# Ighina/MultimodalTopicSegmentation

Measured on AMD Instinct MI355X. Metric: sentences/sec (fwd+bwd), higher is better.
Workload: dtype bf16; 1 GPU; BASELINE configs[1]: restricted-window transformer tagger d=1792 heads=8 ff=256 radius=15 layers=1 focal loss, 64 docs x 256 sentences per GPU, fwd+bwd+Adam(eps 1e-7), inputs resident in HBM; global_batch_docs=64, sentences_per_doc=256, parallelism=dp1 (document-sharded, RCCL all-reduce)

## Files before the change

multimodaltopicsegmentation_amd/csrc/ffn_fused.hip:

```cpp
#include <algorithm>
#include "gemm_common.h"

#define FF_BM 64
#define FF_F 256
#define FF_IMG 32768
#define FF_RING (FF_IMG)
#define FF_A_STAGE (8192 + 32768)
#define FF_B_STAGE 32768
#define FF_LDS (FF_IMG + 4 * FF_B_STAGE)
#ifdef FFN_STAMPS
#define FSTAMP(i) do { const unsigned long long t_ = __builtin_amdgcn_s_memtime(); tacc[i] += t_ - tprev; tprev = t_; } while (0)
#else
#define FSTAMP(i) do { } while (0)
#endif

struct FfnArgs {
  const bf16_t* X;
  const bf16_t* Wa;
  const bf16_t* Wb;
  const float* ba;
  const float* bb;
  const bf16_t* U;
  bf16_t* Uout;
  bf16_t* T;
  bf16_t* Y;
  int M, D, relu;
#ifdef FFN_STAMPS
  unsigned long long* stamps;
#endif
};

__device__ __forceinline__ int ff_col(int j, int n) { return (j >> 1) * 32 + (n >> 2) * 8 + (j & 1) * 4 + (n & 3); }

template <bool PERM>
__device__ __forceinline__ void ff_piece_kmajor(const bf16_t* __restrict__ G, int ld, int row0, int dim, int k0, char* img, int piece, int lane) {
  const int row = piece * 8 + (lane >> 3), pos = lane & 7;
  const int ch = pos ^ ((row >> 1) & 7);
  const int srow = PERM ? (row & ~63) + ff_col((row >> 4) & 3, row & 15) : row;
  const bf16_t* src = G + (size_t)min(row0 + srow, dim - 1) * ld + k0 + ch * 8;
  __builtin_amdgcn_global_load_lds((gptr_t*)src, (lptr_t*)(img + piece * 1024), 16, 0, 0);
}
__device__ __forceinline__ void ff_piece_strided(const bf16_t* __restrict__ G, int ld, int k0, int col0, char* img, int piece, int lane) {
  const int kr = piece * 4 + (lane >> 4), c16 = lane & 15;
  const int ch = ((((c16 >> 1) ^ strided_key(kr))) << 1) | (c16 & 1);
  const bf16_t* src = G + (size_t)(k0 + kr) * ld + col0 + ch * 8;
  __builtin_amdgcn_global_load_lds((gptr_t*)src, (lptr_t*)(img + piece * 1024), 16, 0, 0);
}

__device__ __forceinline__ frag_raw ff_frag_strided(const char* tile, int kbase, int wcol0, int j, int lane) {
  const int r = lane & 15, q = r >> 2, p = r & 3;
  const int col = wcol0 + (j >> 1) * 32 + (j & 1) * 4 + 8 * p;
  const unsigned addr = (unsigned)(uintptr_t)(__attribute__((address_space(3))) const char*)(tile + strided_off(kbase + q, col));
  frag_raw f;
  asm volatile("ds_read_b64_tr_b16 %0, %1" : "=v"(f.lo) : "v"(addr));
  asm volatile("ds_read_b64_tr_b16 %0, %1 offset:1024" : "=v"(f.hi) : "v"(addr));
  return f;
}

#define FF_CWAVES 8
#define FF_LWAVES 4
#define FF_THREADS ((FF_CWAVES + FF_LWAVES) * 64)

template <bool BWD>
__global__ __launch_bounds__(FF_THREADS) void ffn_fused_kernel(const FfnArgs a) {
  constexpr bool WKM = !BWD;
  extern __shared__ __attribute__((aligned(16))) char smem[];
  char* fimg = smem;
  char* ring = smem + FF_RING;
  const int tid = threadIdx.x, lane = tid & 63;
  const int wave = __builtin_amdgcn_readfirstlane(tid >> 6);
  const int bm0 = blockIdx.x * FF_BM;
  const int D = a.D, M = a.M;
  const int nkA = D / 64, nch = D / 256, nB = nch * 4;
#ifdef FFN_STAMPS
  unsigned long long tacc[16] = {0, 0, 0, 0, 0, 0, 0, 0, 0, 0, 0, 0, 0, 0, 0, 0};
  unsigned long long tprev = __builtin_amdgcn_s_memtime();
#define FF_STAMPS_OUT() do { if (a.stamps && lane == 0) for (int i_ = 0; i_ < 16; ++i_) a.stamps[((size_t)blockIdx.x * 12 + wave) * 16 + i_] = tacc[i_]; } while (0)
#else
#define FF_STAMPS_OUT() do { } while (0)
#endif

  if (wave >= FF_CWAVES) {
    const int lw = wave - FF_CWAVES;
    auto dmaA = [&](int kt) {
      char* st = ring + (kt % 3) * FF_A_STAGE;
#pragma unroll
      for (int i = 0; i < 10; ++i) {
        const int q = lw * 10 + i;
        if (q < 8) ff_piece_kmajor<false>(a.X, D, bm0, M, kt * 64, st, q, lane);
        else if constexpr (WKM) ff_piece_kmajor<true>(a.Wa, D, 0, FF_F, kt * 64, st + 8192, q - 8, lane);
        else ff_piece_strided(a.Wa, FF_F, kt * 64, ((q - 8) >> 4) * 128, st + 8192 + ((q - 8) >> 4) * 16384, (q - 8) & 15, lane);
      }
    };
    auto dmaB = [&](int gi) {
      char* st = ring + (gi & 3) * FF_B_STAGE;
      const int c = gi >> 2, kk = gi & 3;
#pragma unroll
      for (int i = 0; i < 8; ++i) {
        const int q = lw * 8 + i;
        if constexpr (WKM) ff_piece_kmajor<true>(a.Wb, FF_F, c * 256, D, kk * 64, st, q, lane);
        else ff_piece_strided(a.Wb, D, kk * 64, c * 256 + (q >> 4) * 128, st + (q >> 4) * 16384, q & 15, lane);
      }
    };
    dmaA(0);
    if (nkA > 1) { dmaA(1); asm volatile("s_waitcnt vmcnt(10)" ::: "memory"); }
    else asm volatile("s_waitcnt vmcnt(0)" ::: "memory");
    __builtin_amdgcn_s_barrier();
#pragma clang loop unroll(disable)
    for (int kt = 0; kt < nkA; ++kt) {
      if (kt + 2 < nkA) { dmaA(kt + 2); FSTAMP(0); asm volatile("s_waitcnt vmcnt(10)" ::: "memory"); }
      else asm volatile("s_waitcnt vmcnt(0)" ::: "memory");
      FSTAMP(3);
      __builtin_amdgcn_s_barrier();
      FSTAMP(4);
    }
    dmaB(0);
    dmaB(1);
    dmaB(2);
    dmaB(3);
    FSTAMP(5);
    asm volatile("s_waitcnt vmcnt(0)" ::: "memory");
    __builtin_amdgcn_s_barrier();
    FSTAMP(6);
#pragma clang loop unroll(disable)
    for (int gi = 0; gi < nB; ++gi) {
      if (gi >= 1 && gi + 3 < nB) { dmaB(gi + 3); FSTAMP(8); asm volatile("s_waitcnt vmcnt(16)" ::: "memory"); }
      else asm volatile("s_waitcnt vmcnt(0)" ::: "memory");
      FSTAMP(11);
      __builtin_amdgcn_s_barrier();
      FSTAMP(12);
    }
    FF_STAMPS_OUT();
    return;
  }

  const int wm = wave >> 2, wn = wave & 3;
  const int r16 = lane & 15, g = lane >> 4;
#ifdef FFN_STAMPS
  int tb = 0;
#endif
  f32x4 acc[2][4];
#pragma unroll
  for (int i = 0; i < 2; ++i)
#pragma unroll
    for (int j = 0; j < 4; ++j) acc[i][j] = (f32x4){0.f, 0.f, 0.f, 0.f};

  const unsigned lds0 = (unsigned)(uintptr_t)(__attribute__((address_space(3))) char*)smem;
  unsigned lk[2];
#pragma unroll
  for (int ks = 0; ks < 2; ++ks) lk[ks] = lds0 + r16 * 128 + (((ks * 4 + g) ^ ((r16 >> 1) & 7)) << 4);
  auto mma_tile = [&](int Aoff, int Boff) {
    LFrag<true> fa[2][2];
    LFrag<WKM> fb[4][2];
#pragma unroll
    for (int ks = 0; ks < 2; ++ks) {
      const unsigned ab = lk[ks] + Aoff + wm * 4096, bb = lk[ks] + Boff + wn * 8192;
#pragma unroll
      for (int j = 0; j < 4; ++j) {
        if constexpr (WKM) asm volatile("ds_read_b128 %0, %1 offset:%2" : "=v"(fb[j][ks].k) : "v"(bb), "n"(j * 2048));
        else fb[j][ks].s = ff_frag_strided(smem + Boff + (wn >> 1) * 16384, ks * 32 + 8 * g, (wn & 1) * 64, j, lane);
      }
#pragma unroll
      for (int i = 0; i < 2; ++i) asm volatile("ds_read_b128 %0, %1 offset:%2" : "=v"(fa[i][ks].k) : "v"(ab), "n"(i * 2048));
    }
    lgkm_wait<0>();
    FSTAMP(tb + 1);
    __builtin_amdgcn_s_setprio(1);
#pragma unroll
    for (int ks = 0; ks < 2; ++ks) {
      bf16x8 vb[4];
#pragma unroll
      for (int j = 0; j < 4; ++j) vb[j] = lfrag_get<WKM>(fb[j][ks]);
#pragma unroll
      for (int i = 0; i < 2; ++i) {
        const bf16x8 va = lfrag_get<true>(fa[i][ks]);
#pragma unroll
        for (int j = 0; j < 4; ++j) acc[i][j] = __builtin_amdgcn_mfma_f32_16x16x32_bf16(vb[j], va, acc[i][j], 0, 0, 0);
      }
    }
    __builtin_amdgcn_s_setprio(0);
    FSTAMP(tb + 2);
  };

  typedef __attribute__((ext_vector_type(4))) unsigned u32x4;
  uint4 upre[2][2];
  float4 b1[2][2];
  if constexpr (BWD) {
#pragma unroll
    for (int i = 0; i < 2; ++i)
#pragma unroll
      for (int h = 0; h < 2; ++h)
        upre[i][h] = *reinterpret_cast<const uint4*>(a.U + (size_t)min(bm0 + wm * 32 + i * 16 + r16, M - 1) * FF_F + wn * 64 + h * 32 + g * 8);
  } else {
#pragma unroll
    for (int h = 0; h < 2; ++h)
#pragma unroll
      for (int e = 0; e < 2; ++e) b1[h][e] = *reinterpret_cast<const float4*>(a.ba + wn * 64 + h * 32 + g * 8 + e * 4);
  }
  __builtin_amdgcn_s_barrier();
#pragma clang loop unroll(disable)
  for (int kt = 0; kt < nkA; ++kt) {
    FSTAMP(0);
    const int st = FF_RING + (kt % 3) * FF_A_STAGE;
    mma_tile(st, st + 8192);
    FSTAMP(3);
    __builtin_amdgcn_s_barrier();
    FSTAMP(4);
  }
#pragma unroll
  for (int i = 0; i < 2; ++i) {
    const int row = wm * 32 + i * 16 + r16;
#pragma unroll
    for (int h = 0; h < 2; ++h) {
      float v[8];
#pragma unroll
      for (int e = 0; e < 4; ++e) { v[e] = acc[i][2 * h][e]; v[4 + e] = acc[i][2 * h + 1][e]; }
      const size_t go = (size_t)(bm0 + row) * FF_F + wn * 64 + h * 32 + g * 8;
      if constexpr (!BWD) {
        v[0] += b1[h][0].x; v[1] += b1[h][0].y; v[2] += b1[h][0].z; v[3] += b1[h][0].w;
        v[4] += b1[h][1].x; v[5] += b1[h][1].y; v[6] += b1[h][1].z; v[7] += b1[h][1].w;
        uint4 pre;
        pre.x = pack_bf16x2(v[0], v[1]); pre.y = pack_bf16x2(v[2], v[3]); pre.z = pack_bf16x2(v[4], v[5]); pre.w = pack_bf16x2(v[6], v[7]);
        *reinterpret_cast<uint4*>(a.Uout + go) = pre;
#pragma unroll
        for (int r = 0; r < 8; ++r) v[r] = a.relu ? fmaxf(v[r], 0.0f) : gelu_erf_f(v[r]);
      } else {
        const unsigned uw[4] = {upre[i][h].x, upre[i][h].y, upre[i][h].z, upre[i][h].w};
#pragma unroll
        for (int r = 0; r < 8; ++r) {
          const float uu = (r & 1) ? bf16_hi(uw[r >> 1]) : bf16_lo(uw[r >> 1]);
          const float dr = to_f32(from_f32<bf16_t>(v[r]));
          v[r] = a.relu ? (uu > 0.0f ? dr : 0.0f) : dr * gelu_erf_grad_f(uu);
        }
      }
      uint4 t;
      t.x = pack_bf16x2(v[0], v[1]); t.y = pack_bf16x2(v[2], v[3]); t.z = pack_bf16x2(v[4], v[5]); t.w = pack_bf16x2(v[6], v[7]);
      *reinterpret_cast<uint4*>(a.T + go) = t;
      *reinterpret_cast<uint4*>(fimg + wn * 8192 + kmajor_off(row, h * 4 + g)) = t;
    }
#pragma unroll
    for (int j = 0; j < 4; ++j) acc[i][j] = (f32x4){0.f, 0.f, 0.f, 0.f};
  }
  FSTAMP(5);
  asm volatile("s_waitcnt lgkmcnt(0)" ::: "memory");
  __builtin_amdgcn_s_barrier();
  FSTAMP(6);
#ifdef FFN_STAMPS
  tb = 8;
#endif

  float4 b2[2][2];
  uint4 res[2][2];
#pragma clang loop unroll(disable)
  for (int c = 0; c < nch; ++c) {
    const int colw = c * 256 + wn * 64 + g * 8;
#pragma unroll
    for (int kk = 0; kk < 4; ++kk) {
      const int gi = c * 4 + kk;
      if (kk == 3) {
        if constexpr (!BWD) {
#pragma unroll
          for (int h = 0; h < 2; ++h)
#pragma unroll
            for (int e = 0; e < 2; ++e) b2[h][e] = *reinterpret_cast<const float4*>(a.bb + colw + h * 32 + e * 4);
        }
      }
      if (kk == 1) {
#pragma unroll
        for (int i = 0; i < 2; ++i)
#pragma unroll
          for (int h = 0; h < 2; ++h)
            res[i][h] = *reinterpret_cast<const uint4*>(a.X + (size_t)min(bm0 + wm * 32 + i * 16 + r16, M - 1) * D + colw + h * 32);
      }
      FSTAMP(8);
      mma_tile(kk * 8192, FF_RING + kk * FF_B_STAGE);
      if (kk == 3) {
#pragma unroll
        for (int i = 0; i < 2; ++i) {
          const int row = bm0 + wm * 32 + i * 16 + r16;
#pragma unroll
          for (int h = 0; h < 2; ++h) {
            float v[8];
#pragma unroll
            for (int e = 0; e < 4; ++e) { v[e] = acc[i][2 * h][e]; v[4 + e] = acc[i][2 * h + 1][e]; }
            if constexpr (!BWD) {
              v[0] += b2[h][0].x; v[1] += b2[h][0].y; v[2] += b2[h][0].z; v[3] += b2[h][0].w;
              v[4] += b2[h][1].x; v[5] += b2[h][1].y; v[6] += b2[h][1].z; v[7] += b2[h][1].w;
            }
            const unsigned rw[4] = {res[i][h].x, res[i][h].y, res[i][h].z, res[i][h].w};
#pragma unroll
            for (int e = 0; e < 4; ++e) { v[2 * e] += bf16_lo(rw[e]); v[2 * e + 1] += bf16_hi(rw[e]); }
            uint4 o;
            o.x = pack_bf16x2(v[0], v[1]); o.y = pack_bf16x2(v[2], v[3]); o.z = pack_bf16x2(v[4], v[5]); o.w = pack_bf16x2(v[6], v[7]);
            *reinterpret_cast<uint4*>(a.Y + (size_t)row * D + colw + h * 32) = o;
          }
#pragma unroll
          for (int j = 0; j < 4; ++j) acc[i][j] = (f32x4){0.f, 0.f, 0.f, 0.f};
        }
      }
      FSTAMP(11);
      __builtin_amdgcn_s_barrier();
      FSTAMP(12);
    }
  }
  FF_STAMPS_OUT();
}

#ifdef FFN_STAMPS
static unsigned long long* g_ffn_stamps = nullptr;
extern "C" void mts_ffn_set_stamps(void* p) { g_ffn_stamps = (unsigned long long*)p; }
#endif
static int ffn_launch(bool bwd, hipStream_t st, const FfnArgs& a0) {
  FfnArgs a = a0;
#ifdef FFN_STAMPS
  a.stamps = g_ffn_stamps;
#endif
  const int grid = ceil_div(a.M, FF_BM);
  if (bwd) {
    auto k = ffn_fused_kernel<true>;
    if (int rc = mts_dyn_lds(k, FF_LDS, "ffn_fused")) return rc;
    hipLaunchKernelGGL(k, dim3(grid), dim3(FF_THREADS), FF_LDS, st, a);
  } else {
    auto k = ffn_fused_kernel<false>;
    if (int rc = mts_dyn_lds(k, FF_LDS, "ffn_fused")) return rc;
    hipLaunchKernelGGL(k, dim3(grid), dim3(FF_THREADS), FF_LDS, st, a);
  }
  MTS_LAUNCH_CHECK("mts_ffn_fused");
  return MTS_OK;
}

static int ffn_check(const char* who, int M, int D, int F, const void* p0, const void* p1, const void* p2, const void* p3, const void* p4) {
  MTS_CHECK_ARG(M > 0 && p0 && p1 && p2 && p3 && p4, "%s: bad arguments", who);
  MTS_UNSUPPORTED(F == FF_F && D >= 256 && D % 256 == 0, "%s: the fused block covers F = 256 and D a multiple of 256 (F=%d, D=%d)", who, F, D);
  return MTS_OK;
}

extern "C" int mts_ffn_supported(int dtype, int M, int D, int F) { return dtype == MTS_BF16 && M > 0 && F == FF_F && D >= 256 && D % 256 == 0; }

extern "C" int mts_ffn_fwd(void* stream, int M, int D, int F, const void* a1, const void* w1, const float* b1, const void* w2, const float* b2,
                           int relu, void* u, void* f, void* s2) {
  if (int rc = ffn_check("mts_ffn_fwd", M, D, F, a1, w1, w2, s2, f)) return rc;
  MTS_CHECK_ARG(b1 && b2 && u, "mts_ffn_fwd: null bias / u");
  FfnArgs a{(const bf16_t*)a1, (const bf16_t*)w1, (const bf16_t*)w2, b1, b2, nullptr, (bf16_t*)u, (bf16_t*)f, (bf16_t*)s2, M, D, relu};
  return ffn_launch(false, (hipStream_t)stream, a);
}

extern "C" int mts_ffn_bwd_data(void* stream, int M, int D, int F, const void* ds2, const void* w1, const void* w2, const void* u, int relu,
                                void* du, void* da1) {
  if (int rc = ffn_check("mts_ffn_bwd_data", M, D, F, ds2, w1, w2, du, da1)) return rc;
  MTS_CHECK_ARG(u, "mts_ffn_bwd_data: null u");
  FfnArgs a{(const bf16_t*)ds2, (const bf16_t*)w2, (const bf16_t*)w1, nullptr, nullptr, (const bf16_t*)u, nullptr, (bf16_t*)du, (bf16_t*)da1, M, D, relu};
  return ffn_launch(true, (hipStream_t)stream, a);
}
```

multimodaltopicsegmentation_amd/csrc/gemm.hip:

```cpp
#include <algorithm>
#include <math.h>
#include <stdlib.h>
#include "common.h"

#include "gemm_common.h"


template <int LAYOUT, typename TC, bool GLDS>
__global__ __launch_bounds__(256, 2) void gemm_bf16_kernel(const GemmArgs a) {
  constexpr bool A_KMAJOR = (LAYOUT == MTS_NT || LAYOUT == MTS_NN);
  constexpr bool B_KMAJOR = (LAYOUT == MTS_NT || LAYOUT == MTS_TT);
  extern __shared__ __attribute__((aligned(16))) char smem[];

  const int tid = threadIdx.x;
  const int lane = tid & 63;
  const int wave = tid >> 6;
  const int wm = wave >> 1, wn = wave & 1;
  const int r16 = lane & 15, g = lane >> 4;

  const int ntn = (a.N + BN - 1) / BN;
  const int ntm = (a.M + BM - 1) / BM;
  const int nt = ntn * ntm;
  int bid = xcd_remap(blockIdx.x, nt);
  const int bm0 = (ntm < ntn ? bid % ntm : bid / ntn) * BM;
// ... 329 lines not shown
      float v[4] = {0.f, 0.f, 0.f, 0.f};
      if (kc) {
        const int row = r0 + (f >> 2), k = k0 + (f & 3) * 4;
        if (row < rdim) {
          const float* p = X + (long)row * sr + k;
          if (vec && k + 3 < kend) { const float4 t = *reinterpret_cast<const float4*>(p); v[0] = t.x; v[1] = t.y; v[2] = t.z; v[3] = t.w; }
          else for (int j = 0; j < 4; ++j) if (k + j < kend) v[j] = p[j];
        }
      } else {
        const int k = k0 + (f >> 5), row = r0 + (f & 31) * 4;
        if (k < kend) {
          const float* p = X + (long)k * sk + row;
          if (vec && row + 3 < rdim) { const float4 t = *reinterpret_cast<const float4*>(p); v[0] = t.x; v[1] = t.y; v[2] = t.z; v[3] = t.w; }
          else for (int j = 0; j < 4; ++j) if (row + j < rdim) v[j] = p[j];
        }
      }
      r[i] = make_float4(v[0], v[1], v[2], v[3]);
    }
  };
  auto store_op = [&](float (&S)[F32_BK][F32_PITCH], bool kc, const float4 (&r)[2]) {
#pragma unroll
    for (int i = 0; i < 2; ++i) {
      const int f = tid + 256 * i;
      if (kc) {
        const int row = f >> 2, k = (f & 3) * 4;
        S[k][row] = r[i].x; S[k + 1][row] = r[i].y; S[k + 2][row] = r[i].z; S[k + 3][row] = r[i].w;
      } else {
        *reinterpret_cast<float4*>(&S[f >> 5][(f & 31) * 4]) = r[i];
      }
    }
  };

  f32x4 acc[4][4];
#pragma unroll
  for (int i = 0; i < 4; ++i)
#pragma unroll
    for (int j = 0; j < 4; ++j) acc[i][j] = (f32x4){0.f, 0.f, 0.f, 0.f};

  const int nk = (kend - kbeg + F32_BK - 1) / F32_BK;
  load_op(A, s.sam, s.sak, a_kc, a_vec, bm0, a.M, kbeg, ra);
  load_op(B, s.sbn, s.sbk, b_kc, b_vec, bn0, a.N, kbeg, rb);
  store_op(As[0], a_kc, ra);
  store_op(Bs[0], b_kc, rb);
  __syncthreads();
  for (int kt = 0; kt < nk; ++kt) {
    const int buf = kt & 1;
    if (kt + 1 < nk) {
      load_op(A, s.sam, s.sak, a_kc, a_vec, bm0, a.M, kbeg + (kt + 1) * F32_BK, ra);
      load_op(B, s.sbn, s.sbk, b_kc, b_vec, bn0, a.N, kbeg + (kt + 1) * F32_BK, rb);
    }
#pragma unroll
    for (int ks = 0; ks < F32_BK / 4; ++ks) {
      float av[4], bv[4];
#pragma unroll
      for (int i = 0; i < 4; ++i) {
        av[i] = As[buf][ks * 4 + g][wm * 64 + i * 16 + r16];
        bv[i] = Bs[buf][ks * 4 + g][wn * 64 + i * 16 + r16];
      }
#pragma unroll
      for (int i = 0; i < 4; ++i)
#pragma unroll
        for (int j = 0; j < 4; ++j) acc[i][j] = __builtin_amdgcn_mfma_f32_16x16x4f32(bv[j], av[i], acc[i][j], 0, 0, 0);
    }
    if (kt + 1 < nk) {
      store_op(As[buf ^ 1], a_kc, ra);
      store_op(Bs[buf ^ 1], b_kc, rb);
    }
    __syncthreads();
  }
#pragma unroll
  for (int i = 0; i < 4; ++i) {
    const int m = bm0 + wm * 64 + i * 16 + r16;
#pragma unroll
    for (int j = 0; j < 4; ++j) {
      const int n = bn0 + wn * 64 + j * 16 + 4 * g;
      float v[4] = {acc[i][j][0], acc[i][j][1], acc[i][j][2], acc[i][j][3]};
      epilogue4<float, float>(a, m, n, v, true);
    }
  }
}

#define COLSUM_RS 128
template <typename T>
__global__ __launch_bounds__(256) void colsum_partial_kernel(const T* __restrict__ X, int M, int N, int ldx,
                                                             float* __restrict__ partial) {
  __shared__ float red[16][64];
  const int cx = threadIdx.x & 15, ry = threadIdx.x >> 4;
  const int n = blockIdx.x * 64 + cx * 4;
  const int rs = blockIdx.y;
  const int rows_per = (M + COLSUM_RS - 1) / COLSUM_RS;
  const int m0 = rs * rows_per, m1 = min(M, m0 + rows_per);
  float s[4] = {0.f, 0.f, 0.f, 0.f};
  if (n + 3 < N) {
    int m = m0 + ry;
    for (; m + 48 < m1; m += 64) {
      float v[4][4];
#pragma unroll
      for (int u = 0; u < 4; ++u) load4<T>(X + (size_t)(m + 16 * u) * ldx + n, v[u]);
#pragma unroll
      for (int u = 0; u < 4; ++u)
#pragma unroll
        for (int i = 0; i < 4; ++i) s[i] += v[u][i];
    }
    for (; m < m1; m += 16) {
      float v[4];
      load4<T>(X + (size_t)m * ldx + n, v);
#pragma unroll
      for (int i = 0; i < 4; ++i) s[i] += v[i];
    }
  } else if (n < N) {
    for (int m = m0 + ry; m < m1; m += 16)
      for (int i = 0; i < 4 && n + i < N; ++i) s[i] += to_f32(X[(size_t)m * ldx + n + i]);
  }
#pragma unroll
  for (int i = 0; i < 4; ++i) red[ry][cx * 4 + i] = s[i];
  __syncthreads();
  if (threadIdx.x < 64) {
    const int c = threadIdx.x, nn = blockIdx.x * 64 + c;
    float t = 0.f;
#pragma unroll
    for (int r = 0; r < 16; ++r) t += red[r][c];
    if (nn < N) partial[(size_t)rs * N + nn] = t;
  }
}
__global__ __launch_bounds__(256) void colsum_final_kernel(const float* __restrict__ partial, int N, int nparts,
                                                           float* __restrict__ out, int accumulate) {
  __shared__ float red[4][64];
  const int col = threadIdx.x & 63, grp = threadIdx.x >> 6;
  const int n = blockIdx.x * 64 + col;
  float s = 0.f;
  if (n < N) {
    int r = grp;
    for (; r + 4 * 7 < nparts; r += 4 * 8) {
      float v[8];
#pragma unroll
      for (int u = 0; u < 8; ++u) v[u] = partial[(size_t)(r + 4 * u) * N + n];
#pragma unroll
      for (int u = 0; u < 8; ++u) s += v[u];
    }
    for (; r < nparts; r += 4) s += partial[(size_t)r * N + n];
  }
  red[grp][col] = s;
  __syncthreads();
  if (grp == 0 && n < N) {
    const float t = (red[0][col] + red[1][col]) + (red[2][col] + red[3][col]);
    out[n] = accumulate ? out[n] + t : t;
  }
}

__global__ __launch_bounds__(256) void splitk_reduce_kernel(const float* __restrict__ slab, int splits, int M, int N, float* __restrict__ C,
                                                            int ldc, int accumulate) {
  const size_t idx = (size_t)blockIdx.x * 256 + threadIdx.x;
  const int n4 = N / 4;
  if (idx >= (size_t)M * n4) return;
  const int m = (int)(idx / n4), n = 4 * (int)(idx % n4);
  float s[4] = {0.f, 0.f, 0.f, 0.f};
  if (accumulate) load4<float>(C + (size_t)m * ldc + n, s);
  const size_t plane = (size_t)M * N;
  for (int z = 0; z < splits; ++z) {
    float v[4];
    load4<float>(slab + z * plane + (size_t)m * N + n, v);
#pragma unroll
    for (int i = 0; i < 4; ++i) s[i] += v[i];
  }
  store4<float>(C + (size_t)m * ldc + n, s);
}

__global__ __launch_bounds__(256) void splitk_reduce_t_kernel(const float* __restrict__ slab, int splits, int M, int N, float* __restrict__ Ct,
                                                              int ldc, int accumulate) {
  __shared__ float tile[32][33];
  const int n0 = blockIdx.x * 32, m0 = blockIdx.y * 32;
  const int tx = threadIdx.x & 31, ty = threadIdx.x >> 5;
  const size_t plane = (size_t)M * N;
#pragma unroll
  for (int r = ty; r < 32; r += 8) {
    const int m = m0 + r, n = n0 + tx;
    float s = 0.f;
    if (m < M && n < N) {
      const float* p = slab + (size_t)m * N + n;
      int z = 0;
      for (; z + 7 < splits; z += 8) {
        float v[8];
#pragma unroll
        for (int u = 0; u < 8; ++u) v[u] = p[(size_t)(z + u) * plane];
#pragma unroll
        for (int u = 0; u < 8; ++u) s += v[u];
      }
      for (; z < splits; ++z) s += p[(size_t)z * plane];
    }
    tile[r][tx] = s;
  }
  __syncthreads();
#pragma unroll
  for (int r = ty; r < 32; r += 8) {
    const int n = n0 + r, m = m0 + tx;
    if (n < N && m < M) {
      float* o = Ct + (size_t)n * ldc + m;
      *o = accumulate ? *o + tile[tx][r] : tile[tx][r];
    }
  }
}

template <typename T> __global__ void cast_kernel(const float* __restrict__ src, T* __restrict__ dst, size_t n) {
  size_t i = ((size_t)blockIdx.x * blockDim.x + threadIdx.x) * 4;
  const size_t stride = (size_t)gridDim.x * blockDim.x * 4;
  for (; i + 3 < n; i += stride) {
    float v[4];
    load4<float>(src + i, v);
    store4<T>(dst + i, v);
  }
  if (i < n && i + 3 >= n)
    for (size_t j = i; j < n; ++j) dst[j] = from_f32<T>(src[j]);
}

template <typename T> __global__ void cast_concat_kernel(const float* __restrict__ s1, const float* __restrict__ s2, T* __restrict__ dst,
                                                          size_t rows, int D1, int D2) {
  const int D = D1 + D2, q = D / 4;
  const size_t total = rows * q;
  for (size_t i = (size_t)blockIdx.x * blockDim.x + threadIdx.x; i < total; i += (size_t)gridDim.x * blockDim.x) {
    const size_t r = i / q;
    const int e = (int)(i - r * q) * 4;
    float v[4];
    load4<float>(e < D1 ? s1 + r * D1 + e : s2 + r * D2 + (e - D1), v);
    store4<T>(dst + r * D + e, v);
  }
}

extern "C" int mts_cast_concat(void* stream, int dst_dtype, size_t rows, int D1, int D2, const float* src1, const float* src2, void* dst) {
  MTS_CHECK_ARG(src1 && src2 && dst && D1 > 0 && D2 > 0 && D1 % 4 == 0 && D2 % 4 == 0, "mts_cast_concat: bad arguments (widths must be multiples of 4)");
  if (rows == 0) return MTS_OK;
  const int blocks = (int)std::min<size_t>(4096, (rows * ((D1 + D2) / 4) + 255) / 256);
  if (dst_dtype == MTS_BF16) hipLaunchKernelGGL(cast_concat_kernel<bf16_t>, dim3(blocks), dim3(256), 0, (hipStream_t)stream, src1, src2, (bf16_t*)dst, rows, D1, D2);
  else if (dst_dtype == MTS_F32) hipLaunchKernelGGL(cast_concat_kernel<float>, dim3(blocks), dim3(256), 0, (hipStream_t)stream, src1, src2, (float*)dst, rows, D1, D2);
  else { mts_set_error("mts_cast_concat: bad dtype %d", dst_dtype); return MTS_ERR_INVALID; }
  MTS_LAUNCH_CHECK("mts_cast_concat");
  return MTS_OK;
}

extern "C" size_t mts_colsum_workspace(int N) { return (size_t)COLSUM_RS * (size_t)N * sizeof(float); }

extern "C" int mts_colsum(void* stream, int dtype, int M, int N, const void* X, int ldx, float* out, int accumulate,
                          void* partial) {
  MTS_CHECK_ARG(M > 0 && N > 0 && X && out && partial, "mts_colsum: bad arguments");
  MTS_CHECK_ARG(dtype == MTS_F32 || dtype == MTS_BF16, "mts_colsum: bad dtype %d", dtype);
  MTS_CHECK_ARG(ldx % 4 == 0, "mts_colsum: ldx must be a multiple of 4");
  hipStream_t st = (hipStream_t)stream;
  const int nparts = min(COLSUM_RS, M);
  dim3 grid(ceil_div(N, 64), COLSUM_RS);
  (void)nparts;
  if (dtype == MTS_F32)
    hipLaunchKernelGGL(colsum_partial_kernel<float>, grid, dim3(256), 0, st, (const float*)X, M, N, ldx, (float*)partial);
  else
    hipLaunchKernelGGL(colsum_partial_kernel<bf16_t>, grid, dim3(256), 0, st, (const bf16_t*)X, M, N, ldx, (float*)partial);
  hipLaunchKernelGGL(colsum_final_kernel, dim3(ceil_div(N, 64)), dim3(256), 0, st, (const float*)partial, N, COLSUM_RS, out,
                     accumulate);
  MTS_LAUNCH_CHECK("mts_colsum");
  return MTS_OK;
}

extern "C" int mts_cast(void* stream, int dst_dtype, const float* src, void* dst, size_t n) {
  MTS_CHECK_ARG(src && dst, "mts_cast: null pointer");
  if (n == 0) return MTS_OK;
  hipStream_t st = (hipStream_t)stream;
  const int blocks = (int)std::min<size_t>(2048, (n / 4 + 255) / 256 + 1);
  if (dst_dtype == MTS_BF16)
    hipLaunchKernelGGL(cast_kernel<bf16_t>, dim3(blocks), dim3(256), 0, st, src, (bf16_t*)dst, n);
  else if (dst_dtype == MTS_F32)
    hipLaunchKernelGGL(cast_kernel<float>, dim3(blocks), dim3(256), 0, st, src, (float*)dst, n);
  else {
    mts_set_error("mts_cast: bad dtype %d", dst_dtype);
    return MTS_ERR_INVALID;
  }
  MTS_LAUNCH_CHECK("mts_cast");
  return MTS_OK;
}

int mts_launch_gemm256(const GemmArgs& a, int layout, bool c_is_f32, int splits, hipStream_t st);
int mts_launch_gemm224(const GemmArgs& a, int layout, bool c_is_f32, int splits, hipStream_t st);
bool mts_gemm224t_applies(const GemmArgs& a, int layout, bool c_is_f32, int splits);

static thread_local int g_gemm_glds = -1;
static thread_local int g_tile_mode = -1;
static thread_local int g_force_splits = 0;
static thread_local int g_tile_order = 1;
static thread_local int g_gemm_deep = 1;
static thread_local int g_chain = 0;
static thread_local int g_combine = 0;
#define MTS_GEMM_WS_HEAD 8192
static thread_local int g_last_tile = 0, g_last_splits = 0;

static thread_local void (*g_mid_hook)(void) = nullptr;
extern "C" int mts_gemm_set_mid_hook(void (*fn)(void)) { g_mid_hook = fn; return MTS_OK; }

extern "C" int mts_gemm_last_plan(int* tile, int* splits) {
  if (tile) *tile = g_last_tile;
  if (splits) *splits = g_last_splits;
  return MTS_OK;
}

void mts_band_set_mfma(int on);
void mts_band_set_fused(int on);
void mts_full_set_mfma(int on);
void mts_t5_set_mfma(int on);
static thread_local int g_f32_mfma = 1;
static thread_local int g_big_min_k = 256;
static thread_local int g_gemm_variant = 0;
void mts_lstm_pair_set_spin_limit(int n);
void mts_lstm_pair_set_max_pairs(int n);
void mts_lstm_pair_set_parts(int n);
extern "C" int mts_set_option(const char* key, int value) {
  if (!key) return MTS_ERR_INVALID;
  if (!strcmp(key, "gemm_tile")) { g_tile_mode = value; return MTS_OK; }
  if (!strcmp(key, "gemm_glds")) { g_gemm_glds = value; return MTS_OK; }
  if (!strcmp(key, "gemm_splits")) { g_force_splits = value; return MTS_OK; }
  if (!strcmp(key, "gemm_order")) { g_tile_order = value; return MTS_OK; }
  if (!strcmp(key, "gemm_chain")) { g_chain = value; return MTS_OK; }
  if (!strcmp(key, "gemm_combine")) { g_combine = value; return MTS_OK; }
  if (!strcmp(key, "gemm_deep")) { g_gemm_deep = value; return MTS_OK; }
  if (!strcmp(key, "gemm_variant")) { g_gemm_variant = value; return MTS_OK; }
  if (!strcmp(key, "gemm_big_min_k")) { g_big_min_k = value; return MTS_OK; }
  if (!strcmp(key, "gemm_f32_mfma")) { g_f32_mfma = value; return MTS_OK; }
  if (!strcmp(key, "band_mfma")) { mts_band_set_mfma(value); return MTS_OK; }
  if (!strcmp(key, "band_fused_bwd")) { mts_band_set_fused(value); return MTS_OK; }
  if (!strcmp(key, "full_mfma")) { mts_full_set_mfma(value); return MTS_OK; }
  if (!strcmp(key, "t5_mfma")) { mts_t5_set_mfma(value); return MTS_OK; }
  if (!strcmp(key, "lstm_pair_spin_limit")) { mts_lstm_pair_set_spin_limit(value); return MTS_OK; }
  if (!strcmp(key, "lstm_pair_max_pairs")) { mts_lstm_pair_set_max_pairs(value); return MTS_OK; }
  if (!strcmp(key, "lstm_parts")) { mts_lstm_pair_set_parts(value); return MTS_OK; }
  mts_set_error("mts_set_option: unknown key %s", key);
  return MTS_ERR_INVALID;
}

template <int LAYOUT, typename TC>
static void launch_bf16(const GemmArgs& a, int splits, hipStream_t st) {
  const int nt = ceil_div(a.M, BM) * ceil_div(a.N, BN);
  if (g_gemm_glds < 0) {
    const char* e = getenv("MTS_GEMM_GLDS");
    g_gemm_glds = (e && e[0] == '0') ? 0 : 1;
  }
  const bool glds = g_gemm_glds && (a.K % BK == 0) && (a.ksplit % BK == 0) && a.M >= 8 && a.N >= 8;
  if (glds) {
    GemmArgs b = a;
    const bool deep = g_gemm_deep && (size_t)nt * splits <= 256 && a.ksplit >= 4 * BK;
    b.nbuf = deep ? 4 : 2;
    auto k = gemm_bf16_kernel<LAYOUT, TC, true>;
    if (deep && mts_dyn_lds(k, 8 * TILE_BYTES, "gemm") != MTS_OK) b.nbuf = 2;
    hipLaunchKernelGGL(k, dim3(nt, 1, splits), dim3(256), (b.nbuf == 4 ? 8 : 4) * TILE_BYTES, st, b);
  } else {
    hipLaunchKernelGGL((gemm_bf16_kernel<LAYOUT, TC, false>), dim3(nt, 1, splits), dim3(256), 4 * TILE_BYTES, st, a);
  }
}

static void plan_bf16(int c_dtype, int layout, int M, int N, int K, unsigned epilogue, bool has_workspace, size_t workspace_bytes,
                      int* use256_out, int* splits_out) {
  if (g_tile_mode < 0) {
    const char* e = getenv("MTS_GEMM_TILE");
    g_tile_mode = e ? atoi(e) : 0;
  }
  const int tile_mode = g_tile_mode;
  const unsigned plain = epilogue & ~MTS_EPI_ACCUM;
  const bool can_split = (c_dtype == MTS_F32 && plain == 0 && has_workspace && N % 4 == 0 && K >= 2048);
  const bool can256 = (K % BK == 0) && K >= g_big_min_k && M >= 8 && N >= 8 && tile_mode != 128;
  const double bw = 3500.0;
  double best = 1e30;
  int splits = 1;
  int use256 = 0;
  const bool can224 = can256 && (N % 224 == 0) && tile_mode != 256;
  for (int big = 0; big <= (can256 ? 2 : 0); ++big) {
    if (big == 2 && !can224) continue;
    if (tile_mode == 256 && can256 && big != 1) continue;
    if (tile_mode == 224 && can224 && big != 2) continue;
    const int tile = big ? 256 : 128;
    const double slots = big ? 256.0 : 512.0;
    const double t_k = layout == MTS_TN ? (big == 2 ? (M % 256 == 0 ? 0.0160 : 0.0200) : big == 1 ? 0.0218 : 0.0145)
                                        : (big ? 0.0232 * (big == 2 ? 0.875 : 1.0) : 0.0180);
    const double t_0 = big ? 7.7 : 6.5;
    const int nt = ceil_div(M, tile) * (big == 2 ? N / 224 : ceil_div(N, tile));
    for (int sp = 1; sp <= (can_split ? 32 : 1); ++sp) {
      const int ks = ceil_div(ceil_div(K, sp), BK) * BK;
      if (ceil_div(K, ks) != sp) continue;
      if (sp > 1 && (size_t)sp * M * N * sizeof(float) > workspace_bytes) break;
      if (g_force_splits > 0 && can_split && sp != g_force_splits) continue;
      const double rounds = ceil((double)nt * sp / slots);
      const double cost = rounds * (ks * t_k + t_0) + (sp > 1 ? (2.0 * sp + 1.0) * M * N * 4.0 / 1e6 / bw : 0.0);
      if (cost < best) { best = cost; splits = sp; use256 = big; }
    }
  }
  *use256_out = use256;
  *splits_out = splits;
}

int mts_gemm224_last_kernel();
int mts_launch_gemm224t_pair(const GemmArgs& a, int splits, const void* A2, const void* B2, float* slab2, hipStream_t st);
bool mts_gemm224t_applies(const GemmArgs& a, int layout, bool c_is_f32, int splits);

static int wgrad_pair_splits(int M, int N, int K, size_t workspace_bytes) {
  if (M % 256 || N % 224 || K % 64 || K < 256) return -1;
  static int cus = 0;
  if (!cus) { int dev = 0; hipDeviceProp_t pr; cus = (hipGetDevice(&dev) == hipSuccess && hipGetDeviceProperties(&pr, dev) == hipSuccess) ? pr.multiProcessorCount : 256; }
  const int nt = (M / 256) * (N / 224);
  int sp = std::max(1, std::min(32, cus / (2 * nt)));
  for (; sp >= 1; --sp) {
    const int ks = ceil_div(ceil_div(K, sp), BK) * BK;
    if (ceil_div(K, ks) != sp) continue;
    if (ks >= 128 && K - (sp - 1) * ks >= 128 && (size_t)2 * sp * M * N * sizeof(float) <= workspace_bytes) return sp;
  }
  return -1;
}
extern "C" size_t mts_wgrad_pair_workspace(int M, int N, int K) {
  const int sp = wgrad_pair_splits(M, N, K, (size_t)-1);
  return sp < 1 ? 0 : (size_t)2 * sp * M * N * sizeof(float);
}
extern "C" int mts_wgrad_pair(void* stream, int M, int N, int K, const void* A1, const void* B1, float* C1, int ldc1, const void* A2, const void* B2,
                              float* C2t, int ldc2t, int lda, int ldb, int accumulate, void* workspace, size_t workspace_bytes) {
  MTS_CHECK_ARG(M > 0 && N > 0 && K > 0 && A1 && B1 && C1 && A2 && B2 && C2t && workspace, "mts_wgrad_pair: bad arguments");
  MTS_CHECK_ARG(ldc1 >= N && ldc2t >= M && ldc1 % 4 == 0, "mts_wgrad_pair: bad output strides");
  const int sp = wgrad_pair_splits(M, N, K, workspace_bytes);
  MTS_UNSUPPORTED(sp >= 1, "mts_wgrad_pair: M=%d N=%d K=%d not covered (M %% 256, N %% 224, K %% 64) or workspace too small", M, N, K);
  hipStream_t st = (hipStream_t)stream;
  GemmArgs a;
  memset(&a, 0, sizeof(a));
  a.A = A1; a.B = B1; a.C = C1;
  a.M = M; a.N = N; a.K = K; a.lda = lda; a.ldb = ldb; a.ldc = ldc1;
  a.epi = 0; a.colscale = 1.0f;
  a.ksplit = ceil_div(ceil_div(K, sp), BK) * BK;
  a.order = 1; a.nbuf = 2; a.variant = 0;
  float* const planes = (float*)workspace;
  a.slab = planes;
  float* const planes2 = planes + (size_t)sp * M * N;
  MTS_UNSUPPORTED(mts_gemm224t_applies(a, MTS_TN, true, sp), "mts_wgrad_pair: operands not covered by the four-wave weight-gradient kernel (alignment / strides)");
  const int rc = mts_launch_gemm224t_pair(a, sp, A2, B2, planes2, st);
  MTS_UNSUPPORTED(rc == MTS_OK, "mts_wgrad_pair: launch refused");
  hipLaunchKernelGGL(splitk_reduce_kernel, dim3((unsigned)(((size_t)M * (N / 4) + 255) / 256)), dim3(256), 0, st, (const float*)planes, sp, M, N, C1, ldc1,
                     accumulate ? 1 : 0);
  hipLaunchKernelGGL(splitk_reduce_t_kernel, dim3(ceil_div(N, 32), ceil_div(M, 32)), dim3(256), 0, st, (const float*)planes2, sp, M, N, C2t, ldc2t,
                     accumulate ? 1 : 0);
  MTS_LAUNCH_CHECK("mts_wgrad_pair");
  return MTS_OK;
}

extern "C" int mts_gemm_plan(int a_dtype, int c_dtype, int layout, int M, int N, int K, unsigned epilogue, size_t workspace_bytes,
                             int* tile, int* splits) {
  MTS_CHECK_ARG(M > 0 && N > 0 && K > 0, "mts_gemm_plan: bad shape M=%d N=%d K=%d", M, N, K);
  MTS_CHECK_ARG(layout == MTS_NT || layout == MTS_NN || layout == MTS_TN || layout == MTS_TT, "mts_gemm_plan: bad layout %d", layout);
  MTS_CHECK_ARG(a_dtype == MTS_F32 || a_dtype == MTS_BF16, "mts_gemm_plan: bad a_dtype %d", a_dtype);
  int use256 = 0, sp = 1;
  const size_t ws_planes = workspace_bytes > MTS_GEMM_WS_HEAD ? workspace_bytes - MTS_GEMM_WS_HEAD : 0;
  if (a_dtype == MTS_BF16) plan_bf16(c_dtype, layout, M, N, K, epilogue, ws_planes > 0, ws_planes, &use256, &sp);
  if (tile) *tile = a_dtype == MTS_F32 ? (g_f32_mfma ? 128 : 64) : use256 == 2 ? 224 : use256 == 1 ? 256 : 128;
  if (splits) *splits = sp;
  return MTS_OK;
}

extern "C" int mts_gemm(void* stream, int a_dtype, int c_dtype, int layout, int M, int N, int K, const void* A, int lda,
                        const void* B, int ldb, void* C, int ldc, const float* bias, const void* residual, int ldr,
                        void* aux, int ldaux, unsigned epilogue, float colscale, int ncols_scaled, void* workspace, size_t workspace_bytes) {
  MTS_CHECK_ARG(M > 0 && N > 0 && K > 0, "mts_gemm: bad shape M=%d N=%d K=%d", M, N, K);
  MTS_CHECK_ARG(A && B && C, "mts_gemm: null operand");
  MTS_CHECK_ARG(layout == MTS_NT || layout == MTS_NN || layout == MTS_TN || layout == MTS_TT, "mts_gemm: bad layout %d", layout);
  MTS_CHECK_ARG(a_dtype == MTS_F32 || a_dtype == MTS_BF16, "mts_gemm: bad a_dtype %d", a_dtype);
  MTS_CHECK_ARG(c_dtype == MTS_F32 || c_dtype == a_dtype, "mts_gemm: c_dtype must be f32 or a_dtype");
  MTS_CHECK_ARG(!(epilogue & MTS_EPI_BIAS) || bias, "mts_gemm: MTS_EPI_BIAS without bias");
  MTS_CHECK_ARG(!(epilogue & MTS_EPI_RESIDUAL) || residual, "mts_gemm: MTS_EPI_RESIDUAL without residual");
  MTS_CHECK_ARG(!(epilogue & MTS_EPI_ACCUM) || c_dtype == MTS_F32, "mts_gemm: MTS_EPI_ACCUM needs fp32 C");
  MTS_CHECK_ARG((epilogue & (MTS_EPI_GELU | MTS_EPI_RELU)) != (MTS_EPI_GELU | MTS_EPI_RELU), "mts_gemm: MTS_EPI_GELU and MTS_EPI_RELU are exclusive");
  hipStream_t st = (hipStream_t)stream;
  GemmArgs a;
  a.A = A; a.B = B; a.C = C; a.bias = bias; a.residual = residual; a.aux = aux;
  a.M = M; a.N = N; a.K = K; a.lda = lda; a.ldb = ldb; a.ldc = ldc; a.ldr = ldr; a.ldaux = ldaux;
  a.epi = epilogue; a.colscale = colscale; a.ncols_scaled = ncols_scaled;
  a.variant = g_gemm_variant;
#ifdef MTS_GEMM_STAMPS
  a.stamps = nullptr;
#endif
  a.ksplit = K; a.slab = nullptr; a.chain = nullptr; a.order = g_tile_order; a.nbuf = 2;

  if (a_dtype == MTS_F32) {
    StrideArgs s;
    if (layout == MTS_NT) { s.sam = lda; s.sak = 1; s.sbn = ldb; s.sbk = 1; }
    else if (layout == MTS_NN) { s.sam = lda; s.sak = 1; s.sbn = 1; s.sbk = ldb; }
    else if (layout == MTS_TT) { s.sam = 1; s.sak = lda; s.sbn = ldb; s.sbk = 1; }
    else { s.sam = 1; s.sak = lda; s.sbn = 1; s.sbk = ldb; }
    MTS_CHECK_ARG(ldc % 4 == 0 && ((uintptr_t)C % 16) == 0, "mts_gemm(f32): C must be 16-byte aligned with ldc %% 4 == 0");
    MTS_CHECK_ARG(!(epilogue & MTS_EPI_RESIDUAL) || (ldr % 4 == 0), "mts_gemm(f32): ldr %% 4");
    const int nt = ceil_div(M, F32_BM) * ceil_div(N, F32_BM);
    int splits = 1;
    if (g_f32_mfma && workspace && !(epilogue & ~MTS_EPI_ACCUM) && N % 4 == 0 && nt <= 128 && K >= 1024) {
      splits = std::min(std::min(16, 256 / nt), K / 512);
      while (splits > 1 && (size_t)splits * M * N * sizeof(float) > workspace_bytes) --splits;
    }
    g_last_tile = 128;
    g_last_splits = splits;
    if (splits > 1) {
      a.ksplit = ceil_div(ceil_div(K, splits), F32_BK) * F32_BK;
      splits = ceil_div(K, a.ksplit);
      a.slab = (float*)workspace;
    }
    if (g_f32_mfma) hipLaunchKernelGGL(gemm_f32_mfma_kernel, dim3(nt, 1, splits), dim3(256), 0, st, a, s);
    else hipLaunchKernelGGL(gemm_f32_kernel, dim3(ceil_div(M, 64) * ceil_div(N, 64)), dim3(256), 0, st, a, s);
    if (splits > 1)
      hipLaunchKernelGGL(splitk_reduce_kernel, dim3((unsigned)(((size_t)M * (N / 4) + 255) / 256)), dim3(256), 0, st, (const float*)workspace,
                         splits, M, N, (float*)C, ldc, (epilogue & MTS_EPI_ACCUM) ? 1 : 0);
    MTS_LAUNCH_CHECK("mts_gemm(f32)");
    return MTS_OK;
  }

  MTS_UNSUPPORTED(lda % 8 == 0 && ldb % 8 == 0 && ((uintptr_t)A % 16) == 0 && ((uintptr_t)B % 16) == 0,
                  "mts_gemm(bf16): A/B must be 16-byte aligned with ld %% 8 == 0 (lda=%d ldb=%d)", lda, ldb);
  if (layout == MTS_NT) MTS_UNSUPPORTED(K % 8 == 0, "mts_gemm(bf16,NT): K %% 8 != 0 (K=%d)", K);
  if (layout == MTS_NN) MTS_UNSUPPORTED(K % 8 == 0 && N % 8 == 0, "mts_gemm(bf16,NN): K,N %% 8 (K=%d N=%d)", K, N);
  if (layout == MTS_TN) MTS_UNSUPPORTED(M % 8 == 0 && N % 8 == 0, "mts_gemm(bf16,TN): M,N %% 8 (M=%d N=%d)", M, N);
  if (layout == MTS_TT) MTS_UNSUPPORTED(M % 8 == 0 && K % 8 == 0, "mts_gemm(bf16,TT): M,K %% 8 (M=%d K=%d)", M, K);
  MTS_UNSUPPORTED(ldc % 4 == 0 && ((uintptr_t)C % (c_dtype == MTS_F32 ? 16 : 8)) == 0, "mts_gemm(bf16): C alignment/ldc");
  MTS_UNSUPPORTED(!(epilogue & MTS_EPI_RESIDUAL) || (ldr % 4 == 0 && ((uintptr_t)residual % 8) == 0), "mts_gemm(bf16): residual alignment");
  MTS_UNSUPPORTED(!aux || (ldaux % 4 == 0 && ((uintptr_t)aux % 8) == 0), "mts_gemm(bf16): aux alignment");

  int splits = 1, use256 = 0;
  const size_t ws_planes = workspace_bytes > MTS_GEMM_WS_HEAD ? workspace_bytes - MTS_GEMM_WS_HEAD : 0;
  float* const planes = workspace ? (float*)((char*)workspace + MTS_GEMM_WS_HEAD) : nullptr;
  plan_bf16(c_dtype, layout, M, N, K, epilogue, workspace != nullptr && ws_planes > 0, ws_planes, &use256, &splits);
  g_last_tile = use256 == 2 ? 224 : use256 == 1 ? 256 : 128;
  g_last_splits = splits;
  a.slab = nullptr;
  bool chained = false;
  if (splits > 1) {
    a.ksplit = ceil_div(ceil_div(K, splits), BK) * BK;
    chained = g_chain && !use256;
    if (chained) {
      const size_t nt128 = (size_t)ceil_div(M, BM) * ceil_div(N, BN);
      a.chain = (unsigned*)planes;
      hipError_t e = hipMemsetAsync(planes, 0, nt128 * sizeof(unsigned), st);
      if (e != hipSuccess) { mts_set_error("mts_gemm: hipMemsetAsync: %s", hipGetErrorString(e)); return MTS_ERR_LAUNCH; }
    } else {
      a.slab = planes;
      if (use256 == 2 && g_combine && (a.variant == 0 || a.variant == 11 || a.variant == 12) && (size_t)ceil_div(M, 256) * (N / 224) * sizeof(unsigned) <= MTS_GEMM_WS_HEAD &&
          mts_gemm224t_applies(a, layout, c_dtype == MTS_F32, splits)) {
        a.chain = (unsigned*)workspace;
        chained = true;
      }
    }
  }
  if (use256) {
    int rc = use256 == 2 ? mts_launch_gemm224(a, layout, c_dtype == MTS_F32, splits, st) : mts_launch_gemm256(a, layout, c_dtype == MTS_F32, splits, st);
    if (rc) return rc;
    if (use256 == 2) g_last_tile = mts_gemm224_last_kernel();
  } else if (c_dtype == MTS_F32) {
    if (layout == MTS_NT) launch_bf16<MTS_NT, float>(a, splits, st);
    else if (layout == MTS_NN) launch_bf16<MTS_NN, float>(a, splits, st);
    else if (layout == MTS_TT) launch_bf16<MTS_TT, float>(a, splits, st);
    else launch_bf16<MTS_TN, float>(a, splits, st);
  } else {
    if (layout == MTS_NT) launch_bf16<MTS_NT, bf16_t>(a, splits, st);
    else if (layout == MTS_NN) launch_bf16<MTS_NN, bf16_t>(a, splits, st);
    else if (layout == MTS_TT) launch_bf16<MTS_TT, bf16_t>(a, splits, st);
    else launch_bf16<MTS_TN, bf16_t>(a, splits, st);
  }
  if (g_mid_hook) g_mid_hook();
  if (splits > 1 && !chained)
    hipLaunchKernelGGL(splitk_reduce_kernel, dim3((unsigned)(((size_t)M * (N / 4) + 255) / 256)), dim3(256), 0, st, (const float*)planes,
                       splits, M, N, (float*)C, ldc, (epilogue & MTS_EPI_ACCUM) ? 1 : 0);
  MTS_LAUNCH_CHECK("mts_gemm(bf16)");
  return MTS_OK;
}
```

Before: 9.440 million sentences/s.

## Stage FFN residual/output through LDS and rotate column-chunk order per block

In the fused FFN kernel, the second-GEMM B ring shrinks from four stages to three. The freed slot becomes an LDS staging tile: loader waves DMA the residual X chunk into it, compute waves add bias and residual there and write the result back in place, and the chunk is stored to global memory with coalesced full-row writes during the next chunk's MMA. Each block also starts its column-chunk loop at a rotated offset, so concurrent blocks read different slices of Wb and avoid hot-spotting the same weight columns. The cost is a shallower prefetch ring and extra lgkmcnt waits and barriers at chunk boundaries.

```diff
diff --git a/multimodaltopicsegmentation_amd/csrc/ffn_fused.hip b/multimodaltopicsegmentation_amd/csrc/ffn_fused.hip
--- a/multimodaltopicsegmentation_amd/csrc/ffn_fused.hip
+++ b/multimodaltopicsegmentation_amd/csrc/ffn_fused.hip
@@ -8,6 +8,10 @@
 #define FF_A_STAGE (8192 + 32768)
 #define FF_B_STAGE 32768
 #define FF_LDS (FF_IMG + 4 * FF_B_STAGE)
+#define FF_STG (FF_IMG + 3 * FF_B_STAGE)
+#define FF_LV_EPI 1
+#define FF_LV_ROTC 2
+#define FF_LV_DEFAULT (FF_LV_EPI | FF_LV_ROTC)
 #ifdef FFN_STAMPS
 #define FSTAMP(i) do { const unsigned long long t_ = __builtin_amdgcn_s_memtime(); tacc[i] += t_ - tprev; tprev = t_; } while (0)
 #else
@@ -57,13 +61,22 @@
   return f;
 }
 
+__device__ __forceinline__ int ff_stg_off(int row, int chunk) { return row * 512 + ((chunk ^ (row & 31)) << 4); }
+__device__ __forceinline__ void ff_piece_stg(const bf16_t* __restrict__ G, int ld, int row0, int dim, int col0, char* stg, int piece, int lane) {
+  const int row = piece * 2 + (lane >> 5), ch = (lane & 31) ^ (row & 31);
+  const bf16_t* src = G + (size_t)min(row0 + row, dim - 1) * ld + col0 + ch * 8;
+  __builtin_amdgcn_global_load_lds((gptr_t*)src, (lptr_t*)(stg + piece * 1024), 16, 0, 0);
+}
+
 #define FF_CWAVES 8
 #define FF_LWAVES 4
 #define FF_THREADS ((FF_CWAVES + FF_LWAVES) * 64)
 
-template <bool BWD>
+template <bool BWD, int LV>
 __global__ __launch_bounds__(FF_THREADS) void ffn_fused_kernel(const FfnArgs a) {
   constexpr bool WKM = !BWD;
+  constexpr bool EPI = LV & FF_LV_EPI, ROTC = LV & FF_LV_ROTC;
+  constexpr int NST = EPI ? 3 : 4;
   extern __shared__ __attribute__((aligned(16))) char smem[];
   char* fimg = smem;
   char* ring = smem + FF_RING;
@@ -72,6 +85,7 @@
   const int bm0 = blockIdx.x * FF_BM;
   const int D = a.D, M = a.M;
   const int nkA = D / 64, nch = D / 256, nB = nch * 4;
+  const int rotc = ROTC ? (int)(blockIdx.x % (unsigned)nch) : 0;
 #ifdef FFN_STAMPS
   unsigned long long tacc[16] = {0, 0, 0, 0, 0, 0, 0, 0, 0, 0, 0, 0, 0, 0, 0, 0};
   unsigned long long tprev = __builtin_amdgcn_s_memtime();
@@ -93,8 +107,10 @@
       }
     };
     auto dmaB = [&](int gi) {
-      char* st = ring + (gi & 3) * FF_B_STAGE;
-      const int c = gi >> 2, kk = gi & 3;
+      char* st = ring + (gi % NST) * FF_B_STAGE;
+      int c = (gi >> 2) + rotc;
+      if (c >= nch) c -= nch;
+      const int kk = gi & 3;
 #pragma unroll
       for (int i = 0; i < 8; ++i) {
         const int q = lw * 8 + i;
@@ -114,18 +130,39 @@
       __builtin_amdgcn_s_barrier();
       FSTAMP(4);
     }
+    auto dmaR = [&](int ci) {
+      int c = ci + rotc;
+      if (c >= nch) c -= nch;
+#pragma unroll
+      for (int i = 0; i < 8; ++i) ff_piece_stg(a.X, D, bm0, M, c * 256, smem + FF_STG, lw * 8 + i, lane);
+    };
     dmaB(0);
     dmaB(1);
     dmaB(2);
-    dmaB(3);
+    if constexpr (EPI) dmaR(0);
+    else dmaB(3);
     FSTAMP(5);
     asm volatile("s_waitcnt vmcnt(0)" ::: "memory");
     __builtin_amdgcn_s_barrier();
     FSTAMP(6);
 #pragma clang loop unroll(disable)
     for (int gi = 0; gi < nB; ++gi) {
-      if (gi >= 1 && gi + 3 < nB) { dmaB(gi + 3); FSTAMP(8); asm volatile("s_waitcnt vmcnt(16)" ::: "memory"); }
-      else asm volatile("s_waitcnt vmcnt(0)" ::: "memory");
+      if constexpr (EPI) {
+        if (gi >= 1 && gi + 2 < nB) {
+          dmaB(gi + 2);
+          if ((gi & 3) == 1 && gi > 4) {
+            dmaR(gi >> 2);
+            FSTAMP(8);
+            asm volatile("s_waitcnt vmcnt(16)" ::: "memory");
+          } else {
+            FSTAMP(8);
+            asm volatile("s_waitcnt vmcnt(8)" ::: "memory");
+          }
+        } else asm volatile("s_waitcnt vmcnt(0)" ::: "memory");
+      } else {
+        if (gi >= 1 && gi + 3 < nB) { dmaB(gi + 3); FSTAMP(8); asm volatile("s_waitcnt vmcnt(16)" ::: "memory"); }
+        else asm volatile("s_waitcnt vmcnt(0)" ::: "memory");
+      }
       FSTAMP(11);
       __builtin_amdgcn_s_barrier();
       FSTAMP(12);
@@ -249,14 +286,24 @@
   tb = 8;
 #endif
 
+  char* stg = smem + FF_STG;
+  auto chunk_out = [&](int c) {
+#pragma unroll
+    for (int t = 0; t < 4; ++t) {
+      const int row = wave * 8 + t * 2 + (lane >> 5), ch = lane & 31;
+      const uint4 o = *reinterpret_cast<const uint4*>(stg + ff_stg_off(row, ch));
+      *reinterpret_cast<uint4*>(a.Y + (size_t)(bm0 + row) * D + c * 256 + ch * 8) = o;
+    }
+  };
   float4 b2[2][2];
   uint4 res[2][2];
+  int slot = 0, cprev = 0;
 #pragma clang loop unroll(disable)
-  for (int c = 0; c < nch; ++c) {
+  for (int ci = 0; ci < nch; ++ci) {
+    const int c = ci + rotc < nch ? ci + rotc : ci + rotc - nch;
     const int colw = c * 256 + wn * 64 + g * 8;
 #pragma unroll
     for (int kk = 0; kk < 4; ++kk) {
-      const int gi = c * 4 + kk;
       if (kk == 3) {
         if constexpr (!BWD) {
 #pragma unroll
@@ -265,7 +312,7 @@
             for (int e = 0; e < 2; ++e) b2[h][e] = *reinterpret_cast<const float4*>(a.bb + colw + h * 32 + e * 4);
         }
       }
-      if (kk == 1) {
+      if (!EPI && kk == 1) {
 #pragma unroll
         for (int i = 0; i < 2; ++i)
 #pragma unroll
@@ -273,7 +320,13 @@
             res[i][h] = *reinterpret_cast<const uint4*>(a.X + (size_t)min(bm0 + wm * 32 + i * 16 + r16, M - 1) * D + colw + h * 32);
       }
       FSTAMP(8);
-      mma_tile(kk * 8192, FF_RING + kk * FF_B_STAGE);
+      if constexpr (EPI) {
+        mma_tile(kk * 8192, FF_RING + slot * FF_B_STAGE);
+        slot = slot == NST - 1 ? 0 : slot + 1;
+        if (kk == 0 && ci > 0) chunk_out(cprev);
+      } else {
+        mma_tile(kk * 8192, FF_RING + kk * FF_B_STAGE);
+      }
       if (kk == 3) {
 #pragma unroll
         for (int i = 0; i < 2; ++i) {
@@ -287,22 +340,28 @@
               v[0] += b2[h][0].x; v[1] += b2[h][0].y; v[2] += b2[h][0].z; v[3] += b2[h][0].w;
               v[4] += b2[h][1].x; v[5] += b2[h][1].y; v[6] += b2[h][1].z; v[7] += b2[h][1].w;
             }
+            uint4* sp = reinterpret_cast<uint4*>(stg + ff_stg_off(wm * 32 + i * 16 + r16, wn * 8 + h * 4 + g));
+            if constexpr (EPI) res[i][h] = *sp;
             const unsigned rw[4] = {res[i][h].x, res[i][h].y, res[i][h].z, res[i][h].w};
 #pragma unroll
             for (int e = 0; e < 4; ++e) { v[2 * e] += bf16_lo(rw[e]); v[2 * e + 1] += bf16_hi(rw[e]); }
             uint4 o;
             o.x = pack_bf16x2(v[0], v[1]); o.y = pack_bf16x2(v[2], v[3]); o.z = pack_bf16x2(v[4], v[5]); o.w = pack_bf16x2(v[6], v[7]);
-            *reinterpret_cast<uint4*>(a.Y + (size_t)row * D + colw + h * 32) = o;
+            if constexpr (EPI) *sp = o;
+            else *reinterpret_cast<uint4*>(a.Y + (size_t)row * D + colw + h * 32) = o;
           }
 #pragma unroll
           for (int j = 0; j < 4; ++j) acc[i][j] = (f32x4){0.f, 0.f, 0.f, 0.f};
         }
       }
       FSTAMP(11);
+      if (EPI && (kk == 0 || kk == 3)) asm volatile("s_waitcnt lgkmcnt(0)" ::: "memory");
       __builtin_amdgcn_s_barrier();
       FSTAMP(12);
     }
-  }
+    cprev = c;
+  }
+  if constexpr (EPI) chunk_out(cprev);
   FF_STAMPS_OUT();
 }
 
@@ -310,23 +369,39 @@
 static unsigned long long* g_ffn_stamps = nullptr;
 extern "C" void mts_ffn_set_stamps(void* p) { g_ffn_stamps = (unsigned long long*)p; }
 #endif
+static thread_local int g_ffn_variant = 1;
+void mts_ffn_set_variant(int v) { g_ffn_variant = v; }
+#ifdef FFN_DBG_LEVERS
+extern "C" void mts_ffn_set_levers(int mask) { g_ffn_variant = mask; }
+#endif
+
+template <bool BWD, int LV>
+static int ffn_launch_as(hipStream_t st, const FfnArgs& a) {
+  auto k = ffn_fused_kernel<BWD, LV>;
+  if (int rc = mts_dyn_lds(k, FF_LDS, "ffn_fused")) return rc;
+  hipLaunchKernelGGL(k, dim3(ceil_div(a.M, FF_BM)), dim3(FF_THREADS), FF_LDS, st, a);
+  MTS_LAUNCH_CHECK("mts_ffn_fused");
+  return MTS_OK;
+}
+template <bool BWD>
+static int ffn_launch_dir(hipStream_t st, const FfnArgs& a) {
+#ifdef FFN_DBG_LEVERS
+  switch (g_ffn_variant & 3) {
+    case 1: return ffn_launch_as<BWD, 1>(st, a);
+    case 2: return ffn_launch_as<BWD, 2>(st, a);
+    case 3: return ffn_launch_as<BWD, 3>(st, a);
+    default: return ffn_launch_as<BWD, 0>(st, a);
+  }
+#else
+  return g_ffn_variant ? ffn_launch_as<BWD, FF_LV_DEFAULT>(st, a) : ffn_launch_as<BWD, 0>(st, a);
+#endif
+}
 static int ffn_launch(bool bwd, hipStream_t st, const FfnArgs& a0) {
   FfnArgs a = a0;
 #ifdef FFN_STAMPS
   a.stamps = g_ffn_stamps;
 #endif
-  const int grid = ceil_div(a.M, FF_BM);
-  if (bwd) {
-    auto k = ffn_fused_kernel<true>;
-    if (int rc = mts_dyn_lds(k, FF_LDS, "ffn_fused")) return rc;
-    hipLaunchKernelGGL(k, dim3(grid), dim3(FF_THREADS), FF_LDS, st, a);
-  } else {
-    auto k = ffn_fused_kernel<false>;
-    if (int rc = mts_dyn_lds(k, FF_LDS, "ffn_fused")) return rc;
-    hipLaunchKernelGGL(k, dim3(grid), dim3(FF_THREADS), FF_LDS, st, a);
-  }
-  MTS_LAUNCH_CHECK("mts_ffn_fused");
-  return MTS_OK;
+  return bwd ? ffn_launch_dir<true>(st, a) : ffn_launch_dir<false>(st, a);
 }
 
 static int ffn_check(const char* who, int M, int D, int F, const void* p0, const void* p1, const void* p2, const void* p3, const void* p4) {
diff --git a/multimodaltopicsegmentation_amd/csrc/gemm.hip b/multimodaltopicsegmentation_amd/csrc/gemm.hip
--- a/multimodaltopicsegmentation_amd/csrc/gemm.hip
+++ b/multimodaltopicsegmentation_amd/csrc/gemm.hip
@@ -655,6 +655,7 @@
 void mts_band_set_fused(int on);
 void mts_full_set_mfma(int on);
 void mts_t5_set_mfma(int on);
+void mts_ffn_set_variant(int v);
 static thread_local int g_f32_mfma = 1;
 static thread_local int g_big_min_k = 256;
 static thread_local int g_gemm_variant = 0;
@@ -677,6 +678,7 @@
   if (!strcmp(key, "band_fused_bwd")) { mts_band_set_fused(value); return MTS_OK; }
   if (!strcmp(key, "full_mfma")) { mts_full_set_mfma(value); return MTS_OK; }
   if (!strcmp(key, "t5_mfma")) { mts_t5_set_mfma(value); return MTS_OK; }
+  if (!strcmp(key, "ffn_variant")) { mts_ffn_set_variant(value); return MTS_OK; }
   if (!strcmp(key, "lstm_pair_spin_limit")) { mts_lstm_pair_set_spin_limit(value); return MTS_OK; }
   if (!strcmp(key, "lstm_pair_max_pairs")) { mts_lstm_pair_set_max_pairs(value); return MTS_OK; }
   if (!strcmp(key, "lstm_parts")) { mts_lstm_pair_set_parts(value); return MTS_OK; }
```

Result: no change. 9.519 million sentences/s, median of 6 (+0.8%).
